# TUMFTM/CamRaDepth

Hardware: AMD Instinct MI355X
Metric: training images/sec at 256x416 bf16 (higher is better)
Workload: dtype bf16; 1 GPU; CamRaDepth base (image+radar) train step, 8x7x256x416 per GPU, bf16 MFMA / fp32 accumulate, diffGradNorm + OneCycleLR, Dropout2d/DropPath on; global_batch=8, parallelism=dp1, hip_graph=True

## Files before the change

camradepth_amd/csrc/encoder_ops.hip:

```cpp
#include <stdlib.h>
#include "common.h"

namespace {

constexpr int TPB = 256;

constexpr int DTH = 8;
constexpr int DCW = 64;

struct InNorm {
  const crd_sum_t* stats;
  const float* gamma; const float* beta; int gmul;
};
__device__ __forceinline__ void innorm_coeffs(const InNorm& n, int b, int C, long long P, int c0, bool ok, float (&a)[8], float (&s)[8]) {
#pragma unroll
  for (int j = 0; j < 8; ++j) { a[j] = 1.f; s[j] = 0.f; }
  if (n.stats == nullptr || !ok) return;
  float mean, rstd;
  const int grp = (c0 >> 4) / n.gmul;
  gn_mean_rstd(n.stats + (long long)b * (C >> 4) * 2, grp * n.gmul, n.gmul, (float)P * 16.f * n.gmul, mean, rstd);
#pragma unroll
  for (int j = 0; j < 8; ++j) {
    a[j] = n.gamma[c0 + j] * rstd;
    s[j] = n.beta[c0 + j] - mean * a[j];
  }
}
__device__ __forceinline__ uint4 innorm_apply(const uint4& u, const float (&a)[8], const float (&s)[8]) {
  uint4 r;
  r.x = pack_bf2(bf_lo(u.x) * a[0] + s[0], bf_hi(u.x) * a[1] + s[1]);
  r.y = pack_bf2(bf_lo(u.y) * a[2] + s[2], bf_hi(u.y) * a[3] + s[3]);
  r.z = pack_bf2(bf_lo(u.z) * a[4] + s[4], bf_hi(u.z) * a[5] + s[5]);
  r.w = pack_bf2(bf_lo(u.w) * a[6] + s[6], bf_hi(u.w) * a[7] + s[7]);
  return r;
}

struct RedOut {
  const bf16_t* xr;
  const crd_sum_t* stats;
  const float* gamma;
  crd_sum_t* r;
};

template <bool FLIP, bool STATS, int TW>
__global__ __launch_bounds__(TPB) void k_dwconv(const bf16_t* x, int H, int W, int C, const float* w9, const float* bias,
                                                bf16_t* y, crd_sum_t* stats, int tiles_x, InNorm inn, RedOut red) {
  constexpr int HWD = TW + 2;
  constexpr int HPX = (DTH + 2) * HWD;
  constexpr int RSPLIT = 32 / TW;
  constexpr int ROWS = DTH / RSPLIT;
  __shared__ __attribute__((aligned(16))) uint4 sh[HPX * 8];
  __shared__ float sred[4][16];
  const int b = blockIdx.z;
  const int c_win = blockIdx.y * DCW;
  const int tyi = blockIdx.x / tiles_x, txi = blockIdx.x - tyi * tiles_x;
  const int ty0 = tyi * DTH, tx0 = txi * TW;
  const bf16_t* xb = x + (long long)b * H * W * C;
  bf16_t* yb = y + (long long)b * H * W * C;
  const int t = threadIdx.x;
  const int nG = (C - c_win) >= DCW ? 8 : (C - c_win) >> 3;
  const int g = t & 7, xc = (t >> 3) % TW, rg = (t >> 3) / TW;
  const int c0 = c_win + g * 8;
  const bool gok = g < nG;
  typedef __attribute__((ext_vector_type(2))) float f32x2;
  f32x2 wv[9][4], bv[4];
  {
    uint4 r[(HPX * 8 + TPB - 1) / TPB];
    bool inimg[(HPX * 8 + TPB - 1) / TPB];
#pragma unroll
    for (int k = 0; k < (HPX * 8 + TPB - 1) / TPB; ++k) {
      const int i = t + k * TPB;
      const int hp = i >> 3, g = i & 7;
      const int hy = hp / HWD, hx = hp - hy * HWD;
      const int iy = ty0 - 1 + hy, ix = tx0 - 1 + hx;
      inimg[k] = i < HPX * 8 && g < nG && (unsigned)iy < (unsigned)H && (unsigned)ix < (unsigned)W;
      const int cy = iy < 0 ? 0 : (iy < H ? iy : H - 1), cx = ix < 0 ? 0 : (ix < W ? ix : W - 1), cgr = g < nG ? g : 0;
      const uint4 u = *reinterpret_cast<const uint4*>(xb + ((long long)cy * W + cx) * C + c_win + cgr * 8);
      r[k] = inimg[k] ? u : make_uint4(0, 0, 0, 0);
    }
#pragma unroll
    for (int tp = 0; tp < 9; ++tp) {
      float w8[8];
      if (gok) load8t<1>(w9, (long long)(FLIP ? 8 - tp : tp) * C + c0, w8);
      else {
#pragma unroll
        for (int j = 0; j < 8; ++j) w8[j] = 0.f;
      }
#pragma unroll
      for (int q = 0; q < 4; ++q) wv[tp][q] = f32x2{w8[2 * q], w8[2 * q + 1]};
    }
#pragma unroll
    for (int q = 0; q < 4; ++q) bv[q] = f32x2{(bias && gok) ? bias[c0 + 2 * q] : 0.f, (bias && gok) ? bias[c0 + 2 * q + 1] : 0.f};
    float na[8], ns[8];
    innorm_coeffs(inn, b, C, (long long)H * W, c_win + (t & 7) * 8, (t & 7) < nG, na, ns);
#pragma unroll
    for (int k = 0; k < (HPX * 8 + TPB - 1) / TPB; ++k) {
      const int i = t + k * TPB;
      if (i < HPX * 8) sh[i] = (inn.stats && inimg[k]) ? innorm_apply(r[k], na, ns) : r[k];
    }
  }
  uint4 xrv[ROWS];
  if (red.xr) {
    const int cgr = gok ? c0 : c_win;
#pragma unroll
    for (int i = 0; i < ROWS; ++i) {
      const int oy = ty0 + rg * ROWS + i, ox = tx0 + xc;
      const int cy = oy < H ? oy : H - 1, cx = ox < W ? ox : W - 1;
      xrv[i] = *reinterpret_cast<const uint4*>(red.xr + (((long long)b * H + cy) * W + cx) * C + cgr);
    }
  }
  __syncthreads();
  auto lds8 = [&](int hy, int hx, f32x2 (&v)[4]) {
    const uint4 u = sh[(hy * HWD + hx) * 8 + g];
    v[0] = f32x2{bf_lo(u.x), bf_hi(u.x)}; v[1] = f32x2{bf_lo(u.y), bf_hi(u.y)};
    v[2] = f32x2{bf_lo(u.z), bf_hi(u.z)}; v[3] = f32x2{bf_lo(u.w), bf_hi(u.w)};
  };
  f32x2 win[3][3][4];
  const int r0 = rg * ROWS;
#pragma unroll
  for (int ky = 0; ky < 2; ++ky)
#pragma unroll
    for (int kx = 0; kx < 3; ++kx) lds8(r0 + ky, xc + kx, win[ky][kx]);
  float s = 0.f, ss = 0.f;
  float rs0[8], rs1[8], rmean = 0.f, rrstd = 0.f;
#pragma unroll
  for (int j = 0; j < 8; ++j) rs0[j] = rs1[j] = 0.f;
  if (red.xr && gok) gn_mean_rstd(red.stats + (long long)b * (C >> 4) * 2, c0 >> 4, 1, (float)H * W * 16.f, rmean, rrstd);
#pragma unroll
  for (int i = 0; i < ROWS; ++i) {
#pragma unroll
    for (int kx = 0; kx < 3; ++kx) lds8(r0 + i + 2, xc + kx, win[(i + 2) % 3][kx]);
    const int oy = ty0 + r0 + i, ox = tx0 + xc;
    f32x2 acc[4];
#pragma unroll
    for (int q = 0; q < 4; ++q) acc[q] = bv[q];
#pragma unroll
    for (int ky = 0; ky < 3; ++ky)
#pragma unroll
      for (int kx = 0; kx < 3; ++kx) {
#pragma unroll
        for (int q = 0; q < 4; ++q) acc[q] = __builtin_elementwise_fma(win[(i + ky) % 3][kx][q], wv[ky * 3 + kx][q], acc[q]);
      }
    if (gok && oy < H && ox < W) {
      uint4 u;
      u.x = pack_bf2(acc[0][0], acc[0][1]); u.y = pack_bf2(acc[1][0], acc[1][1]); u.z = pack_bf2(acc[2][0], acc[2][1]); u.w = pack_bf2(acc[3][0], acc[3][1]);
      *reinterpret_cast<uint4*>(yb + ((long long)oy * W + ox) * C + c0) = u;
      if (red.xr) {
        const uint4 xv = xrv[i];
        const float gq[8] = {bf_lo(u.x), bf_hi(u.x), bf_lo(u.y), bf_hi(u.y), bf_lo(u.z), bf_hi(u.z), bf_lo(u.w), bf_hi(u.w)};
        const float xq[8] = {bf_lo(xv.x), bf_hi(xv.x), bf_lo(xv.y), bf_hi(xv.y), bf_lo(xv.z), bf_hi(xv.z), bf_lo(xv.w), bf_hi(xv.w)};
#pragma unroll
        for (int j = 0; j < 8; ++j) { rs0[j] += gq[j]; rs1[j] += gq[j] * ((xq[j] - rmean) * rrstd); }
      }
      if (STATS) {
        s += bf_lo(u.x) + bf_hi(u.x) + bf_lo(u.y) + bf_hi(u.y) + bf_lo(u.z) + bf_hi(u.z) + bf_lo(u.w) + bf_hi(u.w);
        ss += bf_lo(u.x) * bf_lo(u.x) + bf_hi(u.x) * bf_hi(u.x) + bf_lo(u.y) * bf_lo(u.y) + bf_hi(u.y) * bf_hi(u.y) +
              bf_lo(u.z) * bf_lo(u.z) + bf_hi(u.z) * bf_hi(u.z) + bf_lo(u.w) * bf_lo(u.w) + bf_hi(u.w) * bf_hi(u.w);
      }
    }
  }
  if (STATS) {
    s += __shfl_xor(s, 1); ss += __shfl_xor(ss, 1);
#pragma unroll
    for (int o = 8; o < 64; o <<= 1) { s += __shfl_xor(s, o); ss += __shfl_xor(ss, o); }
    const int wave = t >> 6, l = t & 63;
    if (l < 8 && (l & 1) == 0) { sred[wave][(l >> 1) * 2] = s; sred[wave][(l >> 1) * 2 + 1] = ss; }
    __syncthreads();
    if (t < 8) {
      const float v = sred[0][t] + sred[1][t] + sred[2][t] + sred[3][t];
      const int slab = (c_win >> 4) + (t >> 1);
      if (slab < (C >> 4)) stat_add(&stats[((long long)b * (C >> 4) + slab) * 2 + (t & 1)], v);
    }
  }
  if (red.xr) {
#pragma unroll
    for (int o = 8; o < 64; o <<= 1) {
#pragma unroll
      for (int j = 0; j < 8; ++j) { rs0[j] += __shfl_xor(rs0[j], o); rs1[j] += __shfl_xor(rs1[j], o); }
    }
    __syncthreads();
    float* fr = reinterpret_cast<float*>(sh);
    const int wave = t >> 6, l = t & 63;
    if (l < 8) {
#pragma unroll
      for (int j = 0; j < 8; ++j) { fr[wave * 128 + (l * 8 + j) * 2] = rs0[j]; fr[wave * 128 + (l * 8 + j) * 2 + 1] = rs1[j]; }
    }
    __syncthreads();
    const int nch = nG * 8;
    if (t < 2 * nch) {
      const float v = fr[t] + fr[128 + t] + fr[256 + t] + fr[384 + t];
      const int c = c_win + (t >> 1);
      grad_add(&red.r[((long long)b * C + c) * 2 + (t & 1)], v);
      fr[512 + t] = v * red.gamma[c];
    }
    __syncthreads();
    if (t < 2 * (nch >> 4)) {
      const int grp = t >> 1, which = t & 1;
      float a = 0.f;
#pragma unroll
      for (int j = 0; j < 16; ++j) a += fr[512 + (grp * 16 + j) * 2 + which];
      grad_add(&red.r[(long long)gridDim.z * C * 2 + ((long long)b * (C >> 4) + (c_win >> 4) + grp) * 2 + which], a);
    }
  }
}

#ifndef CRD_DWW_WGS
#define CRD_DWW_WGS 2
#endif
template <int TW>
__global__ __launch_bounds__(TPB, CRD_DWW_WGS) void k_dwconv_wgrad(const bf16_t* x, const bf16_t* dy, int H, int W, int C, crd_sum_t* dw10,
                                                      int replicas, int tiles_x, int tiles_y, int tiles_per_wg, InNorm inn) {
  constexpr int HWD = TW + 2;
  constexpr int HPX = (DTH + 2) * HWD;
  constexpr int RSPLIT = 32 / TW;
  constexpr int ROWS = DTH / RSPLIT;
  extern __shared__ __attribute__((aligned(16))) uint4 dsm[];
  uint4* sx = dsm;
  uint4* sdy = dsm + HPX * 8;
  const int b = blockIdx.z;
  const int c_win = blockIdx.y * DCW;
  const int txi = blockIdx.x % tiles_x, ygrp = blockIdx.x / tiles_x;
  const int tx0 = txi * TW;
  const bf16_t* xb = x + (long long)b * H * W * C;
  const bf16_t* db = dy + (long long)b * H * W * C;
  const int t = threadIdx.x;
  const int nG = (C - c_win) >= DCW ? 8 : (C - c_win) >> 3;
  const int g = t & 7, xc = (t >> 3) % TW, rg = (t >> 3) / TW;
  float acc[10][8];
#pragma unroll
  for (int tp = 0; tp < 10; ++tp)
#pragma unroll
    for (int j = 0; j < 8; ++j) acc[tp][j] = 0.f;
  float na[8], ns[8];
  for (int it = 0; it < tiles_per_wg; ++it) {
    const int tyi = ygrp * tiles_per_wg + it;
    if (tyi >= tiles_y) break;
// ... 67 lines not shown
  __syncthreads();
  float* sm = reinterpret_cast<float*>(dsm);
  const int wave = t >> 6, l = t & 63;
  for (int w = 0; w < 4; ++w) {
    if (wave == w && l < 8) {
#pragma unroll
      for (int tp = 0; tp < 10; ++tp)
#pragma unroll
        for (int j = 0; j < 8; ++j) {
          float* p = &sm[tp * 64 + l * 8 + j];
          *p = w == 0 ? acc[tp][j] : *p + acc[tp][j];
        }
    }
    __syncthreads();
  }
  crd_sum_t* dst = dw10 + (long long)((blockIdx.z * gridDim.x + blockIdx.x) % replicas) * 10 * C;
  const int nch = nG * 8;
  for (int i = t; i < 10 * nch; i += TPB) {
    const int tp = i / nch, cl = i - tp * nch;
    const float v = sm[tp * 64 + cl];
    if (v != 0.f) grad_add(&dst[(long long)tp * C + c_win + cl], v);
  }
}

}

static int dw_tile_width(int W) {
  static int forced = -1;
  if (forced < 0) forced = crd_dev_int("CRD_DW_TW", 0);
  if (forced == 16 || forced == 32) return forced;
  return W <= 16 ? 16 : 32;
}

extern "C" int crd_dwconv3x3(const void* x, int32_t B, int32_t H, int32_t W, int32_t C, const float* w9, const float* bias,
                             int32_t flip, void* y, crd_sum_t* stats, const crd_sum_t* in_stats, int32_t in_gmul,
                             const float* in_gamma, const float* in_beta, const void* red_x, const crd_sum_t* red_stats,
                             const float* red_gamma, crd_sum_t* red_r, crd_stream_t stream) {
  CRD_CHECK_ARG(x && w9 && y, "crd_dwconv3x3: null pointer");
  CRD_CHECK_ARG(!red_x || (red_stats && red_gamma && red_r), "crd_dwconv3x3: incomplete fused-reduce arguments");
  const RedOut red{reinterpret_cast<const bf16_t*>(red_x), red_stats, red_gamma, red_r};
  CRD_CHECK_ARG(!in_stats || (in_gamma && in_beta && in_gmul >= 1 && (C / 16) % in_gmul == 0), "crd_dwconv3x3: bad input-norm arguments");
  const InNorm inn{in_stats, in_gamma, in_beta, in_gmul};
  CRD_CHECK_ARG(C % 16 == 0, "crd_dwconv3x3: C must be a multiple of 16");
  const bf16_t* xp = reinterpret_cast<const bf16_t*>(x);
  bf16_t* yp = reinterpret_cast<bf16_t*>(y);
  hipStream_t st = as_stream(stream);
  const int tw = dw_tile_width(W);
  const int tiles_x = cdiv(W, tw), tiles_y = cdiv(H, DTH);
  dim3 grid(tiles_x * tiles_y, cdiv(C, DCW), B);
#define CRD_DW(FL, STT, TWV) hipLaunchKernelGGL((k_dwconv<FL, STT, TWV>), grid, dim3(TPB), 0, st, xp, H, W, C, w9, bias, yp, stats, tiles_x, inn, red)
  if (tw == 32) {
    if (flip) { if (stats) CRD_DW(true, true, 32); else CRD_DW(true, false, 32); }
    else { if (stats) CRD_DW(false, true, 32); else CRD_DW(false, false, 32); }
  } else {
    if (flip) { if (stats) CRD_DW(true, true, 16); else CRD_DW(true, false, 16); }
    else { if (stats) CRD_DW(false, true, 16); else CRD_DW(false, false, 16); }
  }
#undef CRD_DW
  CRD_LAUNCH_CHECK("crd_dwconv3x3");
  return CRD_OK;
}

extern "C" int crd_dwconv3x3_wgrad(const void* x, const void* dy, int32_t B, int32_t H, int32_t W, int32_t C, crd_sum_t* dw10,
                                   int32_t replicas, const crd_sum_t* in_stats, int32_t in_gmul, const float* in_gamma,
                                   const float* in_beta, crd_stream_t stream) {
  CRD_CHECK_ARG(x && dy && dw10 && replicas >= 1, "crd_dwconv3x3_wgrad: null pointer / replicas < 1");
  CRD_CHECK_ARG(!in_stats || (in_gamma && in_beta && in_gmul >= 1 && (C / 16) % in_gmul == 0), "crd_dwconv3x3_wgrad: bad input-norm arguments");
  const InNorm inn{in_stats, in_gamma, in_beta, in_gmul};
  CRD_CHECK_ARG(C % 16 == 0 && C <= 4096, "crd_dwconv3x3_wgrad: C must be a multiple of 16, <= 4096");
  const int tw = dw_tile_width(W);
  const int tiles_x = cdiv(W, tw), tiles_y = cdiv(H, DTH), wins = cdiv(C, DCW);
  int ysplit = cdiv(512, (long long)tiles_x * wins * B);
  if (ysplit > tiles_y) ysplit = tiles_y;
  if (ysplit < 1) ysplit = 1;
  const int per = cdiv(tiles_y, ysplit);
  ysplit = cdiv(tiles_y, per);
  dim3 grid(tiles_x * ysplit, wins, B);
  const bf16_t* xp = reinterpret_cast<const bf16_t*>(x);
  const bf16_t* dp = reinterpret_cast<const bf16_t*>(dy);
  hipStream_t st = as_stream(stream);
  if (tw == 32) {
    const size_t lds = (size_t)((DTH + 2) * 34 * 8 + DTH * 32 * 8) * sizeof(uint4);
    crd_reserve_lds_once<&k_dwconv_wgrad<32>>((int)lds, "k_dwconv_wgrad");
    hipLaunchKernelGGL(k_dwconv_wgrad<32>, grid, dim3(TPB), lds, st, xp, dp, H, W, C, dw10, replicas, tiles_x, tiles_y, per, inn);
  } else {
    const size_t lds = (size_t)((DTH + 2) * 18 * 8 + DTH * 16 * 8) * sizeof(uint4);
    crd_reserve_lds_once<&k_dwconv_wgrad<16>>((int)lds, "k_dwconv_wgrad");
    hipLaunchKernelGGL(k_dwconv_wgrad<16>, grid, dim3(TPB), lds, st, xp, dp, H, W, C, dw10, replicas, tiles_x, tiles_y, per, inn);
  }
  CRD_LAUNCH_CHECK("crd_dwconv3x3_wgrad");
  return CRD_OK;
// ... 2 lines not shown
```

camradepth_amd/lib.py:

```python
import ctypes as C
import os
import struct

import torch

_HERE = os.path.dirname(os.path.abspath(__file__))
LIB_PATH = os.environ.get("CRD_LIB") or os.path.join(_HERE, "libcamradepth_hip.so")


class CrdError(RuntimeError):
    pass


class ConvDesc(C.Structure):
    _fields_ = [
        ("x", C.c_void_p), ("x_ld", C.c_int32), ("x_coff", C.c_int32),
        ("B", C.c_int32), ("IH", C.c_int32), ("IW", C.c_int32), ("Cin", C.c_int32),
        ("w", C.c_void_p), ("Cout", C.c_int32), ("KH", C.c_int32), ("KW", C.c_int32),
        ("stride", C.c_int32), ("pad", C.c_int32), ("OH", C.c_int32), ("OW", C.c_int32),
        ("gather_mode", C.c_int32),
        ("y", C.c_void_p), ("y_ld", C.c_int32), ("y_coff", C.c_int32), ("y_f32", C.c_int32),
        ("out_mode", C.c_int32), ("patch_k", C.c_int32), ("patch_c", C.c_int32),
        ("bias", C.c_void_p), ("bias_bstride", C.c_int32), ("act", C.c_int32),
        ("res", C.c_void_p), ("res_ld", C.c_int32), ("res_scale", C.c_void_p),
# ... 76 lines not shown
    if not os.path.exists(LIB_PATH):
        raise CrdError(f"{LIB_PATH} is missing: run `python -m camradepth_amd.build` (hipcc, gfx950). "
                       "camradepth_amd has no CPU fallback.")
    lib = C.CDLL(LIB_PATH)
    lib.crd_last_error.restype = C.c_char_p
    lib.crd_arch.restype = C.c_char_p
    lib.crd_version.restype = C.c_int
    if lib.crd_version() != ABI_VERSION:
        raise CrdError(f"{LIB_PATH} was built for ABI version {lib.crd_version()}, this binding is version {ABI_VERSION}: rebuild it "
                       "(python -m camradepth_amd.build)")
    missing = [n for n in EXPORTS if not hasattr(lib, n)]
    if missing:
        raise CrdError(f"{LIB_PATH} lacks symbols {missing}: rebuild it (python -m camradepth_amd.build)")
    for name, sig in _SIGS.items():
        fn = getattr(lib, name)
        fn.restype = C.c_int
        fn.argtypes = [_CT[ch] for ch in sig]
    if os.environ.get("CRD_DEV_SWITCHES") == "1":
        if os.environ.get("CRD_TUNE_REGE") is not None:
            lib.crd_tune_igemm_reg_epilogue(int(os.environ["CRD_TUNE_REGE"]))
        if os.environ.get("CRD_TUNE_NARROW") is not None:
            lib.crd_tune_pw_narrow(int(os.environ["CRD_TUNE_NARROW"]))
    _lib = lib
    return lib


_SIGS = {
    "crd_conv_igemm": "pp", "crd_conv_igemm_route": "ppi", "crd_gn_conv": "ppp", "crd_gn_conv2": "ppppp", "crd_gn_bwd_conv": "ppp", "crd_pw_narrow_supported": "iii", "crd_tune_pw_narrow": "i", "crd_conv3x3_fp8": "ppfp", "crd_amax_bf16": "pliiipp", "crd_quant_fp8": "pliiipiifp",
    "crd_weight_quant_fp8": "piiiippp", "crd_conv3x3_fp8_dgrad": "pppp", "crd_gn_bwd_apply_fp8": "piiipiiiiiipippipppppiipiippp",
    "crd_fp8_scale_update": "ppifip", "crd_quant_fp8_dev": "pliiipiipp", "crd_tune_conv3x3_small_grid": "i", "crd_tune_igemm_reg_epilogue": "i", "crd_conv_wgrad": "pp", "crd_conv_wgrad_splits": "p", "crd_conv_wgrad_route": "ppi", "crd_wgrad_group_build": "piplp", "crd_conv_wgrad_grouped": "ppp",
    "crd_gn_stats": "piiiiiippp", "crd_gn_apply": "piiiiiipippipPiiip".replace("P", "p"),
    "crd_gn_bwd_reduce": "piiipiiiiiipippippplp", "crd_gn_bwd_apply": "piiipiiiiiipippipppppiiiipipp",
    "crd_gn_launch_shape": "iiiippp",
    "crd_dwconv3x3": "piiiippipppippppppp", "crd_dwconv3x3_wgrad": "ppiiiipipippp",
    "crd_attn_scores": "ppiiiiifppp", "crd_attn_scores_fp8": "ppiiiiffppp", "crd_attn_fwd": "ppiiiiifpppppppppp", "crd_attn_xbar": "ppppiiipp", "crd_attn_xbar_proj": "pppppiiippp", "crd_attn_vec_bwd": "ppiiifppp", "crd_attn_out_residual": "pppppiiipp", "crd_attn_out_residual_stats": "pppppiiippp",
    "crd_attn_out_bwd": "ppppiiipppp", "crd_attn_out_bwd_blocks": "iii", "crd_attn_out_bwd_gn": "ppppiiippppppppppp", "crd_attn_scores_bwd": "ppppiiiiifpppp", "crd_attn_bwd": "ppppiiiiifpppppifppp", "crd_attn_scores_bwd_partials": "iiiii", "crd_sum_partials_bf16": "pilplp", "crd_gsum_to_bf16": "pplp",
    "crd_attn_bwd_fused_supported": "iiiii", "crd_attn_bwd_fused": "ppppppp" "iiiii" "f" "ppppp" "ppppppp" "p", "crd_attn_dk_fold": "pilpl" "pp" "iii" "f" "pp" "p",
    "crd_bicubic2x": "piiiiiipiip", "crd_bicubic2x_fp8": "piiiiiipiifpiip", "crd_gn_apply_fp8": "piiiiiipippippiifpiip", "crd_bicubic2x_bwd": "piiiiiipiiip",
    "crd_input_grad": "ppppiiiiiipp",
    "crd_nchw_to_pm": "piiiipiiip", "crd_pm_to_nchw": "piiiiiiipp", "crd_seg_argmax": "piiiiipiiip", "crd_scale_f32": "pplfp",
    "crd_slice_copy": "piipiiliip", "crd_f32_to_bf16_rows": "pipiiliplpiip", "crd_dropout_masks": "ppiiLpp", "crd_sigmoid_bwd": "pplp", "crd_head_conv2_fwd": "pppiiippiip", "crd_head_conv2_bwd": "ppiippiiippip", "crd_head_conv2_bwd_data": "ppiippiiipp", "crd_head_conv2_wgrad": "ppiipiiipip",
    "crd_weight_pack": "pilp", "crd_wgrad_unpack": "pilip",
    "crd_assemble_input": "pppiiifpp", "crd_gt_pyramid": "piiifppppp",
    "crd_augment_draw": "ppiiiiifffffffiLLp", "crd_augment_lut": "piipp", "crd_augment_assemble": "pppppppiiiiifppppp",
    "crd_augment_gather": "ppppiiiiiippppp", "crd_gt_pyramid_from_full": "piiipppp",
    "crd_radar_project": "pppiipppipiiiffpppppppp", "crd_radar_rasterize": "ppppppppiipiiiiiplppp",
    "crd_lidar_project": "pppiippppippipppipiiiffLLpppppppppp", "crd_lidar_ground_truth": "pppppppppiipiiiiipppipLplpppp",
    "crd_depth_unproject": "piiiiipipiiLLLipppppp", "crd_point_cloud": "piiiiipipiiLLLipppipplpppppp",
    "crd_bev_grid": "ppppiiipiLLLiiLLiiiplppppppp",
    "crd_occupancy_update": "pppiiipipipiiiiLiLLLLiiiiiipppppplpppppp",
    "crd_distance_field": "piiiiiippplppppp", "crd_field_paths": "pppiipLpppiiiiiippppppp",
    "crd_nav_field": "piiippipLiiipppp", "crd_nav_paths": "ppiipLppiiipppppp",
    "crd_map_objects": "piiiiiiipLplpppppp",
    "crd_track_objects": "pppp" "iiiii" "LLLL" "ii" "ppppppppp" "p",
    "crd_match_scan": "ppp" "iii" "pipi" "iii" "LLLL" "i" "ppp" "ii" "p" "il" "pl" "ppppppp" "p",
    "crd_plan_rollouts": "pppp" "iiii" "pLpp" "iiii" "ppp" "iii" "LL" "pLL" "iiiii" "pl" "pppp" "ppppp" "p" "p",
    "crd_viz_range": "piiiiipplpp", "crd_viz_draw": "piiiippffipiiffipllp", "crd_seg_labels": "piiiipp",
    "crd_camera_frontend": "piiiilliiippip",
    "crd_resize_nearest_u8":"piiiipiip", "crd_resize_labels_nearest": "piiiipiip", "crd_seg_confusion": "ppiilppp",
    "crd_masked_l1_fwd": "pplpp", "crd_test_metrics": "ppilffpp", "crd_depth_eval": "ppilfffipp", "crd_masked_l1_bwd": "pplppfpp", "crd_ce_fwd": "ppiilpp",
    "crd_ce_focal_bwd": "ppiilppfpp",
    "crd_masked_dist_fwd": "pplpp", "crd_masked_dist_bwd": "pplppfipp", "crd_masked_berhu_max": "pplppp",
    "crd_masked_berhu": "pplppLppfpp", "crd_smoothness_fwd": "ppiiiipp", "crd_smoothness_bwd": "ppiiiippfpp",
    "crd_diffgradnorm_norm": "pp", "crd_diffgradnorm_commit": "pp", "crd_diffgradnorm_step": "pp",
    "crd_mlp_fused_supported": "iiii", "crd_mlp_fwd": "pp", "crd_mlp_reduce": "pipppiiipppp",
    "crd_nonfinite_status": "ip", "crd_nonfinite_capture": "pp",
    "crd_swap_f32": "pplp",
# ... 35 lines not shown
        v = torch.full_like(v, float("nan"))
    return v


def f64_bits(x):
    return struct.unpack("<Q", struct.pack("<d", float(x)))[0]


def check(rc, what=""):
    if rc != 0:
        msg = load().crd_last_error().decode()
        raise CrdError(f"{what} failed with status {rc}: {msg}")


def conv_route(desc):
    buf = C.create_string_buffer(96)
    check(load().crd_conv_igemm_route(C.byref(desc), buf, len(buf)), "crd_conv_igemm_route")
    return buf.value.decode()


def wgrad_route(desc):
    buf = C.create_string_buffer(96)
    check(load().crd_conv_wgrad_route(C.byref(desc), buf, len(buf)), "crd_conv_wgrad_route")
    return buf.value.decode()


def gn_launch_shape(P, Cn, B, kind):
    out = (C.c_int32 * 3)()
    ptr = [C.cast(C.byref(out, 4 * i), C.c_void_p) for i in range(3)]
    check(load().crd_gn_launch_shape(P, Cn, B, kind, *ptr), "crd_gn_launch_shape")
    return out[0], out[1], out[2]


def stream():
    return C.c_void_p(torch.cuda.current_stream().cuda_stream)


def ptr(t):
    return None if t is None else C.c_void_p(t.data_ptr())
```

include/camradepth_hip.h:

```cpp
#ifndef CAMRADEPTH_HIP_H
#define CAMRADEPTH_HIP_H

#include <stdint.h>

#ifdef __cplusplus
extern "C" {
#endif

typedef void* crd_stream_t;

#define CRD_OK 0
#define CRD_E_INVALID (-1)
#define CRD_E_UNSUPPORTED (-2)
#define CRD_E_LAUNCH (-3)

typedef int64_t crd_sum_t;
#define CRD_STAT_FRAC_BITS 20
#define CRD_GRAD_FRAC_BITS 44
int crd_nonfinite_status(int32_t reset, crd_stream_t stream);
int crd_nonfinite_capture(int32_t* window_flag, crd_stream_t stream);

const char* crd_last_error(void);
#define CRD_ABI_VERSION 13
int crd_version(void);
// ... 105 lines not shown
  int32_t n_problems;
  int32_t n_items[4];
  int32_t item_offset[4];
  int64_t bytes;
} crd_wgrad_group_info;
int crd_wgrad_group_build(const crd_wgrad_desc* descs, int32_t n, void* host_table, int64_t capacity,
                          crd_wgrad_group_info* info);
int crd_conv_wgrad_grouped(const void* dev_table, const crd_wgrad_group_info* info, crd_stream_t stream);

int crd_gn_stats(const void* x, int32_t x_f32, int32_t x_ld, int32_t x_coff, int32_t B, int32_t P, int32_t C,
                 crd_sum_t* stats, crd_sum_t* chan_sums, crd_stream_t stream);

int crd_gn_apply(const void* x, int32_t x_f32, int32_t x_ld, int32_t x_coff, int32_t B, int32_t P, int32_t C,
                 const crd_sum_t* stats, int32_t gmul, const float* gamma, const float* beta, int32_t act,
                 const float* mask, void* y, int32_t y_f32, int32_t y_ld, int32_t y_coff, crd_stream_t stream);

int crd_gn_bwd_reduce(const void* x, int32_t x_f32, int32_t x_ld, int32_t x_coff, const void* dy, int32_t dy_f32,
                      int32_t dy_ld, int32_t dy_coff, int32_t B, int32_t P, int32_t C, const crd_sum_t* stats,
                      int32_t gmul, const float* gamma, const float* beta, int32_t act, const float* mask,
                      crd_sum_t* r, float* scratch, int64_t scratch_capacity, crd_stream_t stream);
int crd_gn_bwd_apply(const void* x, int32_t x_f32, int32_t x_ld, int32_t x_coff, const void* dy, int32_t dy_f32,
                     int32_t dy_ld, int32_t dy_coff, int32_t B, int32_t P, int32_t C, const crd_sum_t* stats,
                     int32_t gmul, const float* gamma, const float* beta, int32_t act, const float* mask,
                     const crd_sum_t* r, float* dgamma, float* dbeta, void* dx, int32_t dx_f32, int32_t dx_ld,
                     int32_t dx_coff, int32_t dx_accumulate, void* dx2, int32_t dx2_ld, const float* scale2,
                     crd_stream_t stream);
int crd_gn_launch_shape(int32_t P, int32_t C, int32_t B, int32_t kind, int32_t* nblk, int32_t* chunk, int32_t* batch_pixels);


int crd_dwconv3x3(const void* x, int32_t B, int32_t H, int32_t W, int32_t C, const float* w9, const float* bias,
                  int32_t flip, void* y, crd_sum_t* stats, const crd_sum_t* in_stats, int32_t in_gmul, const float* in_gamma,
                  const float* in_beta, const void* red_x, const crd_sum_t* red_stats, const float* red_gamma, crd_sum_t* red_r,
                  crd_stream_t stream);
int crd_dwconv3x3_wgrad(const void* x, const void* dy, int32_t B, int32_t H, int32_t W, int32_t C, crd_sum_t* dw10,
                        int32_t replicas, const crd_sum_t* in_stats, int32_t in_gmul, const float* in_gamma,
                        const float* in_beta, crd_stream_t stream);

typedef struct {
  const float* x1; const crd_sum_t* x1_stats; const float* norm_gamma; const float* norm_beta;
  const void* w_fc1; const float* b_fc1; const float* norm1_gamma; const float* norm1_beta;
  const float* w9; const float* b_dw; const float* norm2_gamma; const float* norm2_beta;
  const void* w_fc2;
  void* xn; void* h1; void* h2; void* h3;
  crd_sum_t* h1_stats; crd_sum_t* h2_stats;
  float* fc2_partials;
  int32_t B, H, W, C, hidden;
} crd_mlp_desc;
int crd_mlp_fused_supported(int32_t H, int32_t W, int32_t C, int32_t hidden);
int crd_mlp_fwd(const crd_mlp_desc* d, crd_stream_t stream);
int crd_mlp_reduce(const float* fc2_partials, int32_t slabs, const float* x1, const float* b_fc2, const float* dp, int32_t B,
                   int32_t N, int32_t C, float* x2, crd_sum_t* stats, crd_sum_t* chan_sums, crd_stream_t stream);

int crd_attn_scores(const void* q, const void* k, int32_t B, int32_t N, int32_t M, int32_t heads, int32_t d,
                    float scale, float* S, int16_t* idx, crd_stream_t stream);
int crd_attn_scores_fp8(const void* q8, const void* k8, int32_t B, int32_t N, int32_t M, int32_t heads, float qk_scale, float scale,
                        float* ssum, int16_t* idx, crd_stream_t stream);
int crd_attn_fwd(const void* q, const void* k, int32_t B, int32_t N, int32_t M, int32_t heads, int32_t d, float scale,
                 float* S, int16_t* idx, const crd_sum_t* chan_sums, const crd_sum_t* stats, const float* gamma, const float* beta,
                 const void* w_fwd, void* xbar, float* u, crd_stream_t stream);
int crd_attn_xbar(const crd_sum_t* chan_sums, const crd_sum_t* stats, const float* gamma, const float* beta, int32_t B,
                  int32_t N, int32_t C, void* xbar, crd_stream_t stream);
int crd_attn_xbar_proj(const crd_sum_t* chan_sums, const crd_sum_t* stats, const float* gamma, const float* beta, const void* w_fwd,
                       int32_t B, int32_t N, int32_t C, void* xbar, float* u, crd_stream_t stream);
int crd_attn_vec_bwd(const crd_sum_t* t, const void* w_dgrad, int32_t B, int32_t C, int32_t Cpad, float inv_n, void* tb, float* es,
                     crd_stream_t stream);
int crd_attn_out_residual(const float* x, const float* u, const float* S, const float* bp, const float* dp,
// ... 276 lines not shown
```

Before: 477.3 images/s.

## Rewrite depthwise 3x3 conv as register row-streaming kernel with DPP neighbor exchange

Replaces the LDS-tiled depthwise conv with a kernel in which each wave owns 32 channels by 16 columns and streams down a band of rows. Rows are prefetched into a register ring, and horizontal neighbors come from DPP row shifts instead of shared memory. Statistics and the reduction side outputs are reduced with shuffles, with no block barriers. Band height is picked adaptively to fill the GPU. The aim is to drop LDS traffic, syncthreads and halo reloads, at the cost of two halo columns of redundant lanes per 16 and higher register pressure.

Result: no change. 481.6 images/s (median of 6 runs) (+0.9%).

```diff
diff --git a/camradepth_amd/csrc/dwconv_partition.h b/camradepth_amd/csrc/dwconv_partition.h
--- /dev/null
+++ b/camradepth_amd/csrc/dwconv_partition.h
@@ -0,0 +1,24 @@
+#pragma once
+#include <stdint.h>
+
+constexpr int DW_COLS = 14;
+constexpr int DW_CH = 128;
+constexpr int DW_BAND_MAX = 16;
+constexpr int DW_FILL = 256;
+
+struct DwPartition { int32_t band, bands, groups, windows; };
+enum { DW_PART_OK = 0, DW_PART_BAD_SHAPE = 1, DW_PART_OFFSETS = 2, DW_PART_GRID = 3, DW_PART_BAD_BAND = 4 };
+
+static inline int dw_partition(int64_t B, int64_t H, int64_t W, int64_t C, int forced, DwPartition* p) {
+  if (B < 1 || H < 1 || W < 1 || C < 16 || C % 16 != 0) return DW_PART_BAD_SHAPE;
+  if (forced != 0 && forced != 2 && forced != 4 && forced != 8 && forced != 16) return DW_PART_BAD_BAND;
+  if (H > INT32_MAX || W > INT32_MAX || C > INT32_MAX || H * W > INT32_MAX || H * W * C > INT32_MAX) return DW_PART_OFFSETS;
+  const int64_t groups = (W + DW_COLS - 1) / DW_COLS, windows = (C + DW_CH - 1) / DW_CH;
+  int band = forced ? forced : DW_BAND_MAX;
+  if (!forced)
+    while (band > 2 && ((H + band - 1) / band) * groups * windows * B < DW_FILL) band >>= 1;
+  const int64_t bands = (H + band - 1) / band;
+  if (groups * bands > INT32_MAX || windows > 65535 || B > 65535) return DW_PART_GRID;
+  p->band = band; p->bands = (int32_t)bands; p->groups = (int32_t)groups; p->windows = (int32_t)windows;
+  return DW_PART_OK;
+}
diff --git a/camradepth_amd/csrc/encoder_ops.hip b/camradepth_amd/csrc/encoder_ops.hip
--- a/camradepth_amd/csrc/encoder_ops.hip
+++ b/camradepth_amd/csrc/encoder_ops.hip
@@ -1,5 +1,6 @@
 #include <stdlib.h>
 #include "common.h"
+#include "dwconv_partition.h"
 
 namespace {
 
@@ -41,166 +42,178 @@
   crd_sum_t* r;
 };
 
-template <bool FLIP, bool STATS, int TW>
-__global__ __launch_bounds__(TPB) void k_dwconv(const bf16_t* x, int H, int W, int C, const float* w9, const float* bias,
-                                                bf16_t* y, crd_sum_t* stats, int tiles_x, InNorm inn, RedOut red) {
-  constexpr int HWD = TW + 2;
-  constexpr int HPX = (DTH + 2) * HWD;
-  constexpr int RSPLIT = 32 / TW;
-  constexpr int ROWS = DTH / RSPLIT;
-  __shared__ __attribute__((aligned(16))) uint4 sh[HPX * 8];
-  __shared__ float sred[4][16];
+typedef __attribute__((ext_vector_type(2))) float f32x2;
+template <int CTRL>
+__device__ __forceinline__ float dpp_row(float v) {
+  return __int_as_float(__builtin_amdgcn_update_dpp(0, __float_as_int(v), CTRL, 0xf, 0xf, true));
+}
+
+#ifndef CRD_DW_RING
+#define CRD_DW_RING 6
+#endif
+template <bool STATS, bool INNORM, bool RED>
+__global__ __launch_bounds__(TPB, 2) void k_dwconv_rows(const bf16_t* x, int H, int W, int C, const float* w9, const float* bias, int flip,
+                                                        bf16_t* y, crd_sum_t* stats, int groups, int band, InNorm inn, RedOut red) {
+  constexpr int RD = (INNORM && RED) ? 3 : CRD_DW_RING;
+  static_assert(RD % 3 == 0, "the request ring turns with the window ring");
   const int b = blockIdx.z;
-  const int c_win = blockIdx.y * DCW;
-  const int tyi = blockIdx.x / tiles_x, txi = blockIdx.x - tyi * tiles_x;
-  const int ty0 = tyi * DTH, tx0 = txi * TW;
-  const bf16_t* xb = x + (long long)b * H * W * C;
-  bf16_t* yb = y + (long long)b * H * W * C;
-  const int t = threadIdx.x;
-  const int nG = (C - c_win) >= DCW ? 8 : (C - c_win) >> 3;
-  const int g = t & 7, xc = (t >> 3) % TW, rg = (t >> 3) / TW;
-  const int c0 = c_win + g * 8;
-  const bool gok = g < nG;
-  typedef __attribute__((ext_vector_type(2))) float f32x2;
+  const int lane = threadIdx.x & 63, wave = threadIdx.x >> 6;
+  const int c_wave = blockIdx.y * DW_CH + wave * 32;
+  if (c_wave >= C) return;
+  const int col = lane & 15, gr = lane >> 4;
+  const bool gok = c_wave + gr * 8 < C;
+  const int c0 = gok ? c_wave + gr * 8 : c_wave;
+  const int bi = blockIdx.x / groups, gi = blockIdx.x - bi * groups;
+  const int k0 = bi * band, k1 = k0 + band < H ? k0 + band : H;
+  const int n = k1 - k0;
+  const int ox = gi * DW_COLS + col - 1;
+  const bool lane_in = gok && (unsigned)ox < (unsigned)W;
+  const bool writer = lane_in && col >= 1 && col <= DW_COLS;
+  const int cx = ox < 0 ? 0 : (ox < W ? ox : W - 1);
+  const int rstride = W * C, off = cx * C + c0;
+  const bf16_t* xb = x + (long long)b * H * rstride + off;
+  bf16_t* yb = y + (long long)b * H * rstride + off;
+  const bf16_t* xrb = RED ? red.xr + (long long)b * H * rstride + off : nullptr;
+  auto request = [&](const bf16_t* base, int row) {
+    const int cy = row < 0 ? 0 : (row < H ? row : H - 1);
+    return *reinterpret_cast<const uint4*>(base + cy * rstride);
+  };
+  const int last_in = k1 < H ? k1 : H - 1, last_out = k1 - 1;
+  uint4 raw[RD], rx[3];
+#pragma unroll
+  for (int u = 0; u < RD; ++u) raw[u] = request(xb, min(k0 - 1 + u, last_in));
+  if (RED) {
+#pragma unroll
+    for (int u = 0; u < 3; ++u) rx[u] = request(xrb, min(k0 + u, last_out));
+  }
   f32x2 wv[9][4], bv[4];
-  {
-    uint4 r[(HPX * 8 + TPB - 1) / TPB];
-    bool inimg[(HPX * 8 + TPB - 1) / TPB];
-#pragma unroll
-    for (int k = 0; k < (HPX * 8 + TPB - 1) / TPB; ++k) {
-      const int i = t + k * TPB;
-      const int hp = i >> 3, g = i & 7;
-      const int hy = hp / HWD, hx = hp - hy * HWD;
-      const int iy = ty0 - 1 + hy, ix = tx0 - 1 + hx;
-      inimg[k] = i < HPX * 8 && g < nG && (unsigned)iy < (unsigned)H && (unsigned)ix < (unsigned)W;
-      const int cy = iy < 0 ? 0 : (iy < H ? iy : H - 1), cx = ix < 0 ? 0 : (ix < W ? ix : W - 1), cgr = g < nG ? g : 0;
-      const uint4 u = *reinterpret_cast<const uint4*>(xb + ((long long)cy * W + cx) * C + c_win + cgr * 8);
-      r[k] = inimg[k] ? u : make_uint4(0, 0, 0, 0);
-    }
-#pragma unroll
-    for (int tp = 0; tp < 9; ++tp) {
-      float w8[8];
-      if (gok) load8t<1>(w9, (long long)(FLIP ? 8 - tp : tp) * C + c0, w8);
-      else {
-#pragma unroll
-        for (int j = 0; j < 8; ++j) w8[j] = 0.f;
-      }
-#pragma unroll
-      for (int q = 0; q < 4; ++q) wv[tp][q] = f32x2{w8[2 * q], w8[2 * q + 1]};
-    }
-#pragma unroll
-    for (int q = 0; q < 4; ++q) bv[q] = f32x2{(bias && gok) ? bias[c0 + 2 * q] : 0.f, (bias && gok) ? bias[c0 + 2 * q + 1] : 0.f};
-    float na[8], ns[8];
-    innorm_coeffs(inn, b, C, (long long)H * W, c_win + (t & 7) * 8, (t & 7) < nG, na, ns);
-#pragma unroll
-    for (int k = 0; k < (HPX * 8 + TPB - 1) / TPB; ++k) {
-      const int i = t + k * TPB;
-      if (i < HPX * 8) sh[i] = (inn.stats && inimg[k]) ? innorm_apply(r[k], na, ns) : r[k];
-    }
-  }
-  uint4 xrv[ROWS];
-  if (red.xr) {
-    const int cgr = gok ? c0 : c_win;
-#pragma unroll
-    for (int i = 0; i < ROWS; ++i) {
-      const int oy = ty0 + rg * ROWS + i, ox = tx0 + xc;
-      const int cy = oy < H ? oy : H - 1, cx = ox < W ? ox : W - 1;
-      xrv[i] = *reinterpret_cast<const uint4*>(red.xr + (((long long)b * H + cy) * W + cx) * C + cgr);
-    }
-  }
-  __syncthreads();
-  auto lds8 = [&](int hy, int hx, f32x2 (&v)[4]) {
-    const uint4 u = sh[(hy * HWD + hx) * 8 + g];
-    v[0] = f32x2{bf_lo(u.x), bf_hi(u.x)}; v[1] = f32x2{bf_lo(u.y), bf_hi(u.y)};
-    v[2] = f32x2{bf_lo(u.z), bf_hi(u.z)}; v[3] = f32x2{bf_lo(u.w), bf_hi(u.w)};
+#pragma unroll
+  for (int tp = 0; tp < 9; ++tp) {
+    float w8[8];
+    load8t<1>(w9, (long long)(flip ? 8 - tp : tp) * C + c0, w8);
+#pragma unroll
+    for (int q = 0; q < 4; ++q) wv[tp][q] = f32x2{w8[2 * q], w8[2 * q + 1]};
+  }
+#pragma unroll
+  for (int q = 0; q < 4; ++q) bv[q] = bias ? f32x2{bias[c0 + 2 * q], bias[c0 + 2 * q + 1]} : f32x2{0.f, 0.f};
+  float na[8], ns[8];
+  if (INNORM) innorm_coeffs(inn, b, C, (long long)H * W, c0, true, na, ns);
+  float rmean = 0.f, rrstd = 0.f;
+  if (RED) gn_mean_rstd(red.stats + (long long)b * (C >> 4) * 2, c0 >> 4, 1, (float)H * W * 16.f, rmean, rrstd);
+  f32x2 win[3][3][4];
+  auto stage = [&](int row, const uint4& r, f32x2 (&w)[3][4]) {
+    uint4 u = INNORM ? innorm_apply(r, na, ns) : r;
+    const bool in = lane_in && (unsigned)row < (unsigned)H;
+    u.x = in ? u.x : 0u; u.y = in ? u.y : 0u; u.z = in ? u.z : 0u; u.w = in ? u.w : 0u;
+    w[1][0] = f32x2{bf_lo(u.x), bf_hi(u.x)}; w[1][1] = f32x2{bf_lo(u.y), bf_hi(u.y)};
+    w[1][2] = f32x2{bf_lo(u.z), bf_hi(u.z)}; w[1][3] = f32x2{bf_lo(u.w), bf_hi(u.w)};
+#pragma unroll
+    for (int q = 0; q < 4; ++q) {
+      w[0][q] = f32x2{dpp_row<0x111>(w[1][q][0]), dpp_row<0x111>(w[1][q][1])};
+      w[2][q] = f32x2{dpp_row<0x101>(w[1][q][0]), dpp_row<0x101>(w[1][q][1])};
+    }
   };
-  f32x2 win[3][3][4];
-  const int r0 = rg * ROWS;
-#pragma unroll
-  for (int ky = 0; ky < 2; ++ky)
-#pragma unroll
-    for (int kx = 0; kx < 3; ++kx) lds8(r0 + ky, xc + kx, win[ky][kx]);
-  float s = 0.f, ss = 0.f;
-  float rs0[8], rs1[8], rmean = 0.f, rrstd = 0.f;
-#pragma unroll
-  for (int j = 0; j < 8; ++j) rs0[j] = rs1[j] = 0.f;
-  if (red.xr && gok) gn_mean_rstd(red.stats + (long long)b * (C >> 4) * 2, c0 >> 4, 1, (float)H * W * 16.f, rmean, rrstd);
-#pragma unroll
-  for (int i = 0; i < ROWS; ++i) {
-#pragma unroll
-    for (int kx = 0; kx < 3; ++kx) lds8(r0 + i + 2, xc + kx, win[(i + 2) % 3][kx]);
-    const int oy = ty0 + r0 + i, ox = tx0 + xc;
+  stage(k0 - 1, raw[0], win[0]);
+  raw[0] = request(xb, min(k0 - 1 + RD, last_in));
+  stage(k0, raw[1], win[1]);
+  raw[1] = request(xb, min(k0 + RD, last_in));
+#pragma unroll
+  for (int tp = 0; tp < 9; ++tp)
+    asm volatile("" : "+v"(wv[tp][0]), "+v"(wv[tp][1]), "+v"(wv[tp][2]), "+v"(wv[tp][3]));
+  asm volatile("" : "+v"(bv[0]), "+v"(bv[1]), "+v"(bv[2]), "+v"(bv[3]));
+  f32x2 s2 = f32x2{0.f, 0.f}, ss2 = f32x2{0.f, 0.f};
+  f32x2 rs0[4], rs1[4];
+#pragma unroll
+  for (int q = 0; q < 4; ++q) rs0[q] = rs1[q] = f32x2{0.f, 0.f};
+  auto step = [&](int i, bool req, bool req_xr, uint4& r, uint4& xr, const f32x2 (&wa)[3][4], const f32x2 (&wb)[3][4], f32x2 (&wc)[3][4]) {
+    stage(k0 + i + 1, r, wc);
+    if (req) r = request(xb, min(k0 + i + 1 + RD, last_in));
     f32x2 acc[4];
 #pragma unroll
     for (int q = 0; q < 4; ++q) acc[q] = bv[q];
 #pragma unroll
-    for (int ky = 0; ky < 3; ++ky)
+    for (int ky = 0; ky < 3; ++ky) {
+      const f32x2(&wr)[3][4] = ky == 0 ? wa : (ky == 1 ? wb : wc);
 #pragma unroll
       for (int kx = 0; kx < 3; ++kx) {
 #pragma unroll
-        for (int q = 0; q < 4; ++q) acc[q] = __builtin_elementwise_fma(win[(i + ky) % 3][kx][q], wv[ky * 3 + kx][q], acc[q]);
-      }
-    if (gok && oy < H && ox < W) {
-      uint4 u;
-      u.x = pack_bf2(acc[0][0], acc[0][1]); u.y = pack_bf2(acc[1][0], acc[1][1]); u.z = pack_bf2(acc[2][0], acc[2][1]); u.w = pack_bf2(acc[3][0], acc[3][1]);
-      *reinterpret_cast<uint4*>(yb + ((long long)oy * W + ox) * C + c0) = u;
-      if (red.xr) {
-        const uint4 xv = xrv[i];
-        const float gq[8] = {bf_lo(u.x), bf_hi(u.x), bf_lo(u.y), bf_hi(u.y), bf_lo(u.z), bf_hi(u.z), bf_lo(u.w), bf_hi(u.w)};
-        const float xq[8] = {bf_lo(xv.x), bf_hi(xv.x), bf_lo(xv.y), bf_hi(xv.y), bf_lo(xv.z), bf_hi(xv.z), bf_lo(xv.w), bf_hi(xv.w)};
-#pragma unroll
-        for (int j = 0; j < 8; ++j) { rs0[j] += gq[j]; rs1[j] += gq[j] * ((xq[j] - rmean) * rrstd); }
-      }
+        for (int q = 0; q < 4; ++q) acc[q] = __builtin_elementwise_fma(wr[kx][q], wv[ky * 3 + kx][q], acc[q]);
+      }
+    }
+    uint4 o;
+    o.x = pack_bf2(acc[0][0], acc[0][1]); o.y = pack_bf2(acc[1][0], acc[1][1]);
+    o.z = pack_bf2(acc[2][0], acc[2][1]); o.w = pack_bf2(acc[3][0], acc[3][1]);
+    uint4 xv = make_uint4(0, 0, 0, 0);
+    if (RED) {
+      xv = xr;
+      if (req_xr) xr = request(xrb, min(k0 + i + 3, last_out));
+    }
+    if (writer) {
+      *reinterpret_cast<uint4*>(yb + (k0 + i) * rstride) = o;
+      const f32x2 g[4] = {f32x2{bf_lo(o.x), bf_hi(o.x)}, f32x2{bf_lo(o.y), bf_hi(o.y)}, f32x2{bf_lo(o.z), bf_hi(o.z)},
+                          f32x2{bf_lo(o.w), bf_hi(o.w)}};
       if (STATS) {
-        s += bf_lo(u.x) + bf_hi(u.x) + bf_lo(u.y) + bf_hi(u.y) + bf_lo(u.z) + bf_hi(u.z) + bf_lo(u.w) + bf_hi(u.w);
-        ss += bf_lo(u.x) * bf_lo(u.x) + bf_hi(u.x) * bf_hi(u.x) + bf_lo(u.y) * bf_lo(u.y) + bf_hi(u.y) * bf_hi(u.y) +
-              bf_lo(u.z) * bf_lo(u.z) + bf_hi(u.z) * bf_hi(u.z) + bf_lo(u.w) * bf_lo(u.w) + bf_hi(u.w) * bf_hi(u.w);
-      }
-    }
+#pragma unroll
+        for (int q = 0; q < 4; ++q) { s2 += g[q]; ss2 = __builtin_elementwise_fma(g[q], g[q], ss2); }
+      }
+      if (RED) {
+        const f32x2 xq[4] = {f32x2{bf_lo(xv.x), bf_hi(xv.x)}, f32x2{bf_lo(xv.y), bf_hi(xv.y)}, f32x2{bf_lo(xv.z), bf_hi(xv.z)},
+                             f32x2{bf_lo(xv.w), bf_hi(xv.w)}};
+#pragma unroll
+        for (int q = 0; q < 4; ++q) {
+          rs0[q] += g[q];
+          rs1[q] = __builtin_elementwise_fma(g[q], (xq[q] - f32x2{rmean, rmean}) * f32x2{rrstd, rrstd}, rs1[q]);
+        }
+      }
+    }
+  };
+  auto flush_red = [&]() {
+    float v[16];
+#pragma unroll
+    for (int q = 0; q < 4; ++q) { v[4 * q] = rs0[q][0]; v[4 * q + 1] = rs1[q][0]; v[4 * q + 2] = rs0[q][1]; v[4 * q + 3] = rs1[q][1]; }
+#pragma unroll
+    for (int d = 8; d >= 1; d >>= 1) {
+      const bool hi = (col & d) != 0;
+#pragma unroll
+      for (int k = 0; k < d; ++k) {
+        const float keep = hi ? v[k + d] : v[k], send = hi ? v[k] : v[k + d];
+        v[k] = keep + __shfl_xor(send, d);
+      }
+    }
+    const float gv0 = v[0] * red.gamma[c0 + (col >> 1)];
+    if (gok) grad_add(&red.r[((long long)b * C + c0) * 2 + col], v[0]);
+    float gv = gv0;
+    gv += __shfl_xor(gv, 2); gv += __shfl_xor(gv, 4); gv += __shfl_xor(gv, 8); gv += __shfl_xor(gv, 16);
+    if ((lane & 31) < 2 && gok)
+      grad_add(&red.r[(long long)gridDim.z * C * 2 + ((long long)b * (C >> 4) + (c0 >> 4)) * 2 + col], gv);
+#pragma unroll
+    for (int q = 0; q < 4; ++q) rs0[q] = rs1[q] = f32x2{0.f, 0.f};
+  };
+  constexpr int FU = 7 % RD;
+  const int nm = n - n % RD;
+  for (int i = 0; i < nm; i += RD) {
+#pragma unroll
+    for (int u = 0; u < RD; ++u) {
+      step(i + u, true, true, raw[(u + 2) % RD], rx[u % 3], win[u % 3], win[(u + 1) % 3], win[(u + 2) % 3]);
+      if (RED && u == FU && i == 7 - FU && n > 8) flush_red();
+    }
+  }
+#pragma unroll
+  for (int u = 0; u < RD - 1; ++u) {
+    if (nm + u >= n) break;
+    step(nm + u, false, RD > 3, raw[(u + 2) % RD], rx[u % 3], win[u % 3], win[(u + 1) % 3], win[(u + 2) % 3]);
+    if (RED && u == FU && nm == 7 - FU && n > 8) flush_red();
   }
   if (STATS) {
-    s += __shfl_xor(s, 1); ss += __shfl_xor(ss, 1);
-#pragma unroll
-    for (int o = 8; o < 64; o <<= 1) { s += __shfl_xor(s, o); ss += __shfl_xor(ss, o); }
-    const int wave = t >> 6, l = t & 63;
-    if (l < 8 && (l & 1) == 0) { sred[wave][(l >> 1) * 2] = s; sred[wave][(l >> 1) * 2 + 1] = ss; }
-    __syncthreads();
-    if (t < 8) {
-      const float v = sred[0][t] + sred[1][t] + sred[2][t] + sred[3][t];
-      const int slab = (c_win >> 4) + (t >> 1);
-      if (slab < (C >> 4)) stat_add(&stats[((long long)b * (C >> 4) + slab) * 2 + (t & 1)], v);
-    }
-  }
-  if (red.xr) {
-#pragma unroll
-    for (int o = 8; o < 64; o <<= 1) {
-#pragma unroll
-      for (int j = 0; j < 8; ++j) { rs0[j] += __shfl_xor(rs0[j], o); rs1[j] += __shfl_xor(rs1[j], o); }
-    }
-    __syncthreads();
-    float* fr = reinterpret_cast<float*>(sh);
-    const int wave = t >> 6, l = t & 63;
-    if (l < 8) {
-#pragma unroll
-      for (int j = 0; j < 8; ++j) { fr[wave * 128 + (l * 8 + j) * 2] = rs0[j]; fr[wave * 128 + (l * 8 + j) * 2 + 1] = rs1[j]; }
-    }
-    __syncthreads();
-    const int nch = nG * 8;
-    if (t < 2 * nch) {
-      const float v = fr[t] + fr[128 + t] + fr[256 + t] + fr[384 + t];
-      const int c = c_win + (t >> 1);
-      grad_add(&red.r[((long long)b * C + c) * 2 + (t & 1)], v);
-      fr[512 + t] = v * red.gamma[c];
-    }
-    __syncthreads();
-    if (t < 2 * (nch >> 4)) {
-      const int grp = t >> 1, which = t & 1;
-      float a = 0.f;
-#pragma unroll
-      for (int j = 0; j < 16; ++j) a += fr[512 + (grp * 16 + j) * 2 + which];
-      grad_add(&red.r[(long long)gridDim.z * C * 2 + ((long long)b * (C >> 4) + (c_win >> 4) + grp) * 2 + which], a);
-    }
-  }
+    float s = s2[0] + s2[1], ss = ss2[0] + ss2[1];
+#pragma unroll
+    for (int o = 1; o < 32; o <<= 1) { s += __shfl_xor(s, o); ss += __shfl_xor(ss, o); }
+    if ((lane & 31) == 0 && gok) {
+      crd_sum_t* p = stats + ((long long)b * (C >> 4) + (c0 >> 4)) * 2;
+      stat_add(p, s); stat_add(p + 1, ss);
+    }
+  }
+  if (RED) flush_red();
 }
 
 #ifndef CRD_DWW_WGS
@@ -334,6 +347,25 @@
   return W <= 16 ? 16 : 32;
 }
 
+static int g_dw_band = 0;
+
+extern "C" int crd_tune_dwconv_band(int32_t band) {
+  const int prev = g_dw_band;
+  if (band == 0 || band == 2 || band == 4 || band == 8 || band == 16) g_dw_band = band;
+  return prev;
+}
+
+extern "C" int crd_dwconv_launch_shape(int32_t B, int32_t H, int32_t W, int32_t C, int32_t band, int32_t* shape4) {
+  CRD_CHECK_ARG(shape4, "crd_dwconv_launch_shape: null pointer");
+  DwPartition part;
+  const int prc = dw_partition(B, H, W, C, band, &part);
+  CRD_CHECK_ARG(prc != DW_PART_BAD_SHAPE && prc != DW_PART_BAD_BAND,
+                "crd_dwconv_launch_shape: B, H, W >= 1, C a multiple of 16, band 0 (the rule), 2, 4, 8 or 16");
+  CRD_UNSUPPORTED(prc == DW_PART_OK, "crd_dwconv_launch_shape: %d x %d x %d x %d: a sample needs 64-bit offsets, or the grid exceeds its limits", B, H, W, C);
+  shape4[0] = part.band; shape4[1] = part.bands; shape4[2] = part.groups; shape4[3] = part.windows;
+  return CRD_OK;
+}
+
 extern "C" int crd_dwconv3x3(const void* x, int32_t B, int32_t H, int32_t W, int32_t C, const float* w9, const float* bias,
                              int32_t flip, void* y, crd_sum_t* stats, const crd_sum_t* in_stats, int32_t in_gmul,
                              const float* in_gamma, const float* in_beta, const void* red_x, const crd_sum_t* red_stats,
@@ -347,18 +379,17 @@
   const bf16_t* xp = reinterpret_cast<const bf16_t*>(x);
   bf16_t* yp = reinterpret_cast<bf16_t*>(y);
   hipStream_t st = as_stream(stream);
-  const int tw = dw_tile_width(W);
-  const int tiles_x = cdiv(W, tw), tiles_y = cdiv(H, DTH);
-  dim3 grid(tiles_x * tiles_y, cdiv(C, DCW), B);
-#define CRD_DW(FL, STT, TWV) hipLaunchKernelGGL((k_dwconv<FL, STT, TWV>), grid, dim3(TPB), 0, st, xp, H, W, C, w9, bias, yp, stats, tiles_x, inn, red)
-  if (tw == 32) {
-    if (flip) { if (stats) CRD_DW(true, true, 32); else CRD_DW(true, false, 32); }
-    else { if (stats) CRD_DW(false, true, 32); else CRD_DW(false, false, 32); }
-  } else {
-    if (flip) { if (stats) CRD_DW(true, true, 16); else CRD_DW(true, false, 16); }
-    else { if (stats) CRD_DW(false, true, 16); else CRD_DW(false, false, 16); }
-  }
-#undef CRD_DW
+  DwPartition part;
+  const int prc = dw_partition(B, H, W, C, g_dw_band, &part);
+  CRD_CHECK_ARG(prc != DW_PART_BAD_SHAPE, "crd_dwconv3x3: B, H, W >= 1 and C >= 16");
+  CRD_UNSUPPORTED(prc == DW_PART_OK, "crd_dwconv3x3: %d x %d x %d x %d: a sample needs 64-bit offsets, or the grid exceeds its limits", B, H, W, C);
+  const dim3 grid(part.groups * part.bands, part.windows, B);
+  const int key = (stats ? 1 : 0) | (in_stats ? 2 : 0) | (red_x ? 4 : 0);
+#define CRD_DWR(K)                                                                                                                    \
+  case K: hipLaunchKernelGGL((k_dwconv_rows<(K & 1) != 0, (K & 2) != 0, (K & 4) != 0>), grid, dim3(TPB), 0, st, xp, H, W, C, w9, bias, \
+                             flip ? 1 : 0, yp, stats, part.groups, part.band, inn, red); break
+  switch (key) { CRD_DWR(0); CRD_DWR(1); CRD_DWR(2); CRD_DWR(3); CRD_DWR(4); CRD_DWR(5); CRD_DWR(6); CRD_DWR(7); }
+#undef CRD_DWR
   CRD_LAUNCH_CHECK("crd_dwconv3x3");
   return CRD_OK;
 }
diff --git a/camradepth_amd/lib.py b/camradepth_amd/lib.py
--- a/camradepth_amd/lib.py
+++ b/camradepth_amd/lib.py
@@ -132,7 +132,7 @@
     "crd_gn_stats": "piiiiiippp", "crd_gn_apply": "piiiiiipippipPiiip".replace("P", "p"),
     "crd_gn_bwd_reduce": "piiipiiiiiipippippplp", "crd_gn_bwd_apply": "piiipiiiiiipippipppppiiiipipp",
     "crd_gn_launch_shape": "iiiippp",
-    "crd_dwconv3x3": "piiiippipppippppppp", "crd_dwconv3x3_wgrad": "ppiiiipipippp",
+    "crd_dwconv3x3": "piiiippipppippppppp", "crd_dwconv3x3_wgrad": "ppiiiipipippp", "crd_dwconv_launch_shape": "iiiiip", "crd_tune_dwconv_band": "i",
     "crd_attn_scores": "ppiiiiifppp", "crd_attn_scores_fp8": "ppiiiiffppp", "crd_attn_fwd": "ppiiiiifpppppppppp", "crd_attn_xbar": "ppppiiipp", "crd_attn_xbar_proj": "pppppiiippp", "crd_attn_vec_bwd": "ppiiifppp", "crd_attn_out_residual": "pppppiiipp", "crd_attn_out_residual_stats": "pppppiiippp",
     "crd_attn_out_bwd": "ppppiiipppp", "crd_attn_out_bwd_blocks": "iii", "crd_attn_out_bwd_gn": "ppppiiippppppppppp", "crd_attn_scores_bwd": "ppppiiiiifpppp", "crd_attn_bwd": "ppppiiiiifpppppifppp", "crd_attn_scores_bwd_partials": "iiiii", "crd_sum_partials_bf16": "pilplp", "crd_gsum_to_bf16": "pplp",
     "crd_attn_bwd_fused_supported": "iiiii", "crd_attn_bwd_fused": "ppppppp" "iiiii" "f" "ppppp" "ppppppp" "p", "crd_attn_dk_fold": "pilpl" "pp" "iii" "f" "pp" "p",
@@ -234,6 +234,12 @@
     return out[0], out[1], out[2]
 
 
+def dwconv_launch_shape(B, H, W, Cn, band=0):
+    out = (C.c_int32 * 4)()
+    check(load().crd_dwconv_launch_shape(B, H, W, Cn, band, C.cast(out, C.c_void_p)), "crd_dwconv_launch_shape")
+    return tuple(out)
+
+
 def stream():
     return C.c_void_p(torch.cuda.current_stream().cuda_stream)
 
diff --git a/include/camradepth_hip.h b/include/camradepth_hip.h
--- a/include/camradepth_hip.h
+++ b/include/camradepth_hip.h
@@ -161,6 +161,8 @@
                   int32_t flip, void* y, crd_sum_t* stats, const crd_sum_t* in_stats, int32_t in_gmul, const float* in_gamma,
                   const float* in_beta, const void* red_x, const crd_sum_t* red_stats, const float* red_gamma, crd_sum_t* red_r,
                   crd_stream_t stream);
+int crd_dwconv_launch_shape(int32_t B, int32_t H, int32_t W, int32_t C, int32_t band, int32_t* shape4);
+int crd_tune_dwconv_band(int32_t band);
 int crd_dwconv3x3_wgrad(const void* x, const void* dy, int32_t B, int32_t H, int32_t W, int32_t C, crd_sum_t* dw10,
                         int32_t replicas, const crd_sum_t* in_stats, int32_t in_gmul, const float* in_gamma,
                         const float* in_beta, crd_stream_t stream);
```
